# twosixlabs/csl-gan

Hardware: AMD Instinct MI355X
Metric: images/sec/GPU CelebA DCResNet dp_mode=gc bs=128 at 1/2/4/8 MI355X (higher is better)
Workload: dtype f32; 1 GPU; CelebA DCResNet D-step: dp_mode=gc -gcm adaptive-pl -nms 32, WGAN-GP on mean samples, 3x64x64; compute_dtype=fp32_auto, storage_dtype=fp32, launch=hip_graph, batch_per_gpu=128, global_batch=128, parallelism=dp1, materialize=ghost, grad_sample_dtype=fp32, fuse_passes=True

## Files before the change

csl_gan_amd/csrc/igemm_skinny.hip:

```cpp
#include "common.h"
#include "device_prims.h"
#include "igemm.h"
#include "conv_classes.h"

namespace cslgan {

constexpr int SK_MAXT = 9;
constexpr int SK_C = 64;
constexpr int SK_HALO = 12 * 12;

template <int NJ, bool ALL>
__global__ __launch_bounds__(256) void igemm_skinny_kernel(const KcParams p) {
    __shared__ float4 Hs[SK_HALO * 16];

    const int tid = threadIdx.x;
    const int b = xcd_remap(blockIdx.x, p.tiles_m);
    int ci = 0;
    if (!ALL) {
#pragma unroll 1
        while (ci + 1 < p.n_cls && b >= p.cls[ci + 1].tile0) ++ci;
    }
    const KcClass& kc = p.cls[ci];
    const int HW_ = kc.halo_w, hpix = kc.halo_h * kc.halo_w;
    const RowCoord rc0 = kc_decode_row((ALL ? b : b - kc.tile0) * 64, kc.OHc, kc.OWc, 1);
    const int y0 = rc0.oy + kc.ty_min, x0 = rc0.ox + kc.tx_min;
    const int img_base = rc0.img * p.AH * p.AW * SK_C;

    const __amdgpu_buffer_rsrc_t a_rsrc = make_rsrc(p.a, p.a_bytes);
    const int cl = tid & 15;
    if (p.a_bf16) {
        constexpr int HREG8 = (SK_HALO * 8 + 255) / 256;
        uint4 r8[HREG8];
#pragma unroll
        for (int j = 0; j < HREG8; ++j) {
            const int idx = tid + 256 * j;
            const int c8 = idx & 7, pix = idx >> 3;
            const int hy = pix / HW_, hx = pix - hy * HW_;
            const int iy = y0 + hy, ix = x0 + hx;
            const bool ok = pix < hpix && (unsigned)iy < (unsigned)p.VH && (unsigned)ix < (unsigned)p.VW;
            const auto v = buf_load4_raw(a_rsrc, (ok ? 2u * (unsigned)(img_base + (iy * p.AW + ix) * SK_C + c8 * 8) : BUF_OOB));
            r8[j] = make_uint4(v[0], v[1], v[2], v[3]);
        }
#pragma unroll
        for (int j = 0; j < HREG8; ++j) {
            const int idx = tid + 256 * j;
            if ((idx >> 3) < hpix) {
                const uint4 v = r8[j];
                Hs[2 * idx] = make_float4(bf_lo(v.x), bf_hi(v.x), bf_lo(v.y), bf_hi(v.y));
                Hs[2 * idx + 1] = make_float4(bf_lo(v.z), bf_hi(v.z), bf_lo(v.w), bf_hi(v.w));
            }
        }
    } else {
        constexpr int HREG = (SK_HALO * 16 + 255) / 256;
        float4 rh[HREG];
        unsigned okm = 0;
        const bool aff = p.in_scale != nullptr;
        float4 sc = make_float4(1.f, 1.f, 1.f, 1.f), sh = make_float4(0.f, 0.f, 0.f, 0.f);
        if (aff) {
            sc = *reinterpret_cast<const float4*>(p.in_scale + rc0.img * SK_C + cl * 4);
            sh = *reinterpret_cast<const float4*>(p.in_shift + rc0.img * SK_C + cl * 4);
        }
#pragma unroll
        for (int j = 0; j < HREG; ++j) {
            const int idx = tid + 256 * j;
            const int c4 = idx & 15, pix = idx >> 4;
            const int hy = pix / HW_, hx = pix - hy * HW_;
            const int iy = y0 + hy, ix = x0 + hx;
            const bool ok = pix < hpix && (unsigned)iy < (unsigned)p.VH && (unsigned)ix < (unsigned)p.VW;
            okm |= (ok ? 1u : 0u) << j;
            rh[j] = buf_load4(a_rsrc, ok ? 4u * (unsigned)(img_base + (iy * p.AW + ix) * SK_C + c4 * 4) : BUF_OOB);
        }
#pragma unroll
        for (int j = 0; j < HREG; ++j) {
            const int idx = tid + 256 * j;
            if (aff) {
                const float lo = p.in_relu ? 0.f : -__builtin_inff();
                const bool in = (okm >> j) & 1u;
                rh[j].x = in ? fmaxf(fmaf(sc.x, rh[j].x, sh.x), lo) : 0.f;
                rh[j].y = in ? fmaxf(fmaf(sc.y, rh[j].y, sh.y), lo) : 0.f;
                rh[j].z = in ? fmaxf(fmaf(sc.z, rh[j].z, sh.z), lo) : 0.f;
                rh[j].w = in ? fmaxf(fmaf(sc.w, rh[j].w, sh.w), lo) : 0.f;
            }
            if ((idx >> 4) < hpix) Hs[idx] = rh[j];
        }
    }
    __syncthreads();

    const int wid = tid >> 6, pg = (tid & 63) >> 4;
    float bv = 0.f;
    if (p.bias && cl < p.Nn) bv = p.bias[cl];
#pragma unroll 1
    for (int cc = ALL ? 0 : ci; cc < (ALL ? p.n_cls : ci + 1); ++cc) {
    const KcClass& kk = p.cls[cc];
    const int Tc = kk.T;
    const __amdgpu_buffer_rsrc_t w_rsrc = make_rsrc(p.w + kk.w_off, p.w_bytes - 4u * (unsigned)kk.w_off);
    float4 wr[SK_MAXT][NJ];
    int toff[SK_MAXT];
#pragma unroll
    for (int t = 0; t < SK_MAXT; ++t) {
        toff[t] = t < Tc ? (((int)kk.ty[t] - kk.ty_min) * HW_ + ((int)kk.tx[t] - kk.tx_min)) * 16 : 0;
#pragma unroll
        for (int j = 0; j < NJ; ++j)
            wr[t][j] = buf_load4(w_rsrc, (t < Tc && j < p.Nn) ? 4u * (unsigned)(j * kk.Kdim + t * SK_C + cl * 4) : BUF_OOB);
    }
#pragma unroll
    for (int it = 0; it < 4; ++it) {
        const int q = wid * 16 + it * 4 + pg;
        const int qy = q >> 3, qx = q & 7;
        const int base = (qy * HW_ + qx) * 16 + cl;
        float acc[NJ];
#pragma unroll
        for (int j = 0; j < NJ; ++j) acc[j] = 0.f;
#pragma unroll
        for (int t = 0; t < SK_MAXT; ++t) {
            if (t < Tc) {
                const float4 a = Hs[base + toff[t]];
#pragma unroll
                for (int j = 0; j < NJ; ++j) {
                    acc[j] = fmaf(a.x, wr[t][j].x, acc[j]);
                    acc[j] = fmaf(a.y, wr[t][j].y, acc[j]);
                    acc[j] = fmaf(a.z, wr[t][j].z, acc[j]);
                    acc[j] = fmaf(a.w, wr[t][j].w, acc[j]);
                }
            }
        }
#pragma unroll
        for (int j = 0; j < NJ; ++j) {
            acc[j] += __shfl_xor(acc[j], 1);
            acc[j] += __shfl_xor(acc[j], 2);
            acc[j] += __shfl_xor(acc[j], 4);
            acc[j] += __shfl_xor(acc[j], 8);
        }
        if (cl < p.Nn) {
            float val = acc[0];
#pragma unroll
            for (int j = 1; j < NJ; ++j) val = cl == j ? acc[j] : val;
            val += bv;
            const RowCoord rc = {rc0.img, rc0.oy + qy, rc0.ox + qx};
            const int off = kc_out_offset(p, kk, rc);
            if (p.res) val += p.res[kc_res_offset(p, kk, rc) + cl];
            val = apply_act(val, p.act);
            if (p.mask) val = lrelu_mask(val, p.mask[off + cl]);
            p.out[off + cl] = val;
        }
    }
    }
}

bool skinny_eligible(const KcParams& p) {
    if (p.Nn > 4 || p.Nn < 1 || p.sy != 1 || p.sx != 1 || p.AC != SK_C) return false;
    if (!aligned16(p.a) || !aligned16(p.w)) return false;
    for (int c = 0; c < p.n_cls; ++c) {
        const KcClass& k = p.cls[c];
        if (k.T < 1 || k.T > SK_MAXT || (k.OHc & 7) || (k.OWc & 7) || (k.M & 63) || (k.w_off & 3)) return false;
        int ymin, ymax, xmin, xmax;
        tap_range(k, ymin, ymax, xmin, xmax);
        if (ymax - ymin > 4 || xmax - xmin > 4) return false;
    }
    return true;
}

int launch_skinny(KcParams& p, hipStream_t st) {
    int tm = 0;
    for (int c = 0; c < p.n_cls; ++c) {
        KcClass& k = p.cls[c];
        int ymin, ymax, xmin, xmax;
        tap_range(k, ymin, ymax, xmin, xmax);
        k.ty_min = ymin; k.tx_min = xmin; k.halo_h = 8 + ymax - ymin; k.halo_w = 8 + xmax - xmin;
        k.patch = 1;
        k.tile0 = tm;
        tm += k.M / 64;
    }
    bool all = p.n_cls > 1;
    int uy0 = 127, uy1 = -128, ux0 = 127, ux1 = -128;
    for (int c = 0; c < p.n_cls; ++c) {
        const KcClass& k = p.cls[c];
        all = all && k.OHc == p.cls[0].OHc && k.OWc == p.cls[0].OWc && k.M == p.cls[0].M;
        uy0 = k.ty_min < uy0 ? k.ty_min : uy0; ux0 = k.tx_min < ux0 ? k.tx_min : ux0;
        uy1 = k.ty_min + k.halo_h > uy1 ? k.ty_min + k.halo_h : uy1; ux1 = k.tx_min + k.halo_w > ux1 ? k.tx_min + k.halo_w : ux1;
    }
    all = all && (uy1 - uy0) * (ux1 - ux0) <= SK_HALO;
    if (all) {
        for (int c = 0; c < p.n_cls; ++c) {
            KcClass& k = p.cls[c];
            k.ty_min = uy0; k.tx_min = ux0; k.halo_h = uy1 - uy0; k.halo_w = ux1 - ux0;
        }
        tm = p.cls[0].M / 64;
    }
    p.tiles_m = tm;
    p.tiles_n = 1;
    p.ksplit = 1;
    const dim3 grid((unsigned)tm), block(256);
    note_kernel("igemm_skinny_kernel<%d%s>", p.Nn < 4 ? p.Nn : 4, all ? ",all" : "");
#define CSL_SKINNY(NJ_)                                                                              \
    if (all) hipLaunchKernelGGL((igemm_skinny_kernel<NJ_, true>), grid, block, 0, st, p);            \
    else hipLaunchKernelGGL((igemm_skinny_kernel<NJ_, false>), grid, block, 0, st, p);
    switch (p.Nn) {
        case 1: CSL_SKINNY(1) break;
        case 2: CSL_SKINNY(2) break;
        case 3: CSL_SKINNY(3) break;
        default: CSL_SKINNY(4) break;
    }
#undef CSL_SKINNY
    return check_launch("igemm_skinny_kernel");
}


struct SkinnyWgradParams {
    const float* gy;
    const float* x;
    int N, H, W, P, Q, T, n_patches;
    unsigned x_bytes;
    float alpha;
    float* partial;
    signed char ty[SK_MAXT], tx[SK_MAXT];
    int ty_min, tx_min, halo_h, halo_w;
};

template <int NJ>
__global__ __launch_bounds__(256) void skinny_wgrad_kernel(const SkinnyWgradParams p) {
    __shared__ float4 Hs[SK_HALO * 16];
    __shared__ float Gs[64 * 4];
    const int tid = threadIdx.x;
    const int T = p.T, HW_ = p.halo_w, hpix = p.halo_h * p.halo_w;
    const int cl = tid & 15, wid = tid >> 6, pg = (tid & 63) >> 4;
    const __amdgpu_buffer_rsrc_t x_rsrc = make_rsrc(p.x, p.x_bytes);
    int toff[SK_MAXT];
#pragma unroll
    for (int t = 0; t < SK_MAXT; ++t) toff[t] = t < T ? (((int)p.ty[t] - p.ty_min) * HW_ + ((int)p.tx[t] - p.tx_min)) * 16 : 0;
    float4 acc[SK_MAXT][NJ];
#pragma unroll
    for (int t = 0; t < SK_MAXT; ++t)
#pragma unroll
        for (int j = 0; j < NJ; ++j) acc[t][j] = make_float4(0.f, 0.f, 0.f, 0.f);

    constexpr int HREG = (SK_HALO * 16 + 255) / 256;
    const int per_img = (p.P >> 3) * (p.Q >> 3);
    for (int pt = blockIdx.x; pt < p.n_patches; pt += gridDim.x) {
        const int img = pt / per_img, rem = pt - img * per_img;
        const int gyy = rem / (p.Q >> 3), gxx = rem - gyy * (p.Q >> 3);
        const int oy0 = gyy << 3, ox0 = gxx << 3;
        float4 rh[HREG];
#pragma unroll
        for (int j = 0; j < HREG; ++j) {
            const int idx = tid + 256 * j;
            const int c4 = idx & 15, pix = idx >> 4;
            const int hy = pix / HW_, hx = pix - hy * HW_;
            const int iy = oy0 + p.ty_min + hy, ix = ox0 + p.tx_min + hx;
            const bool ok = pix < hpix && (unsigned)iy < (unsigned)p.H && (unsigned)ix < (unsigned)p.W;
            rh[j] = buf_load4(x_rsrc, ok ? 4u * (unsigned)(((img * p.H + iy) * p.W + ix) * SK_C + c4 * 4) : BUF_OOB);
        }
        float gv = 0.f;
        if (tid < 64 * NJ) {
            const int q = tid / NJ, j = tid - q * NJ;
            gv = p.gy[((long long)(img * p.P + oy0 + (q >> 3)) * p.Q + ox0 + (q & 7)) * NJ + j];
        }
        __syncthreads();
#pragma unroll
        for (int j = 0; j < HREG; ++j) {
            const int idx = tid + 256 * j;
            if ((idx >> 4) < hpix) Hs[idx] = rh[j];
        }
        if (tid < 64 * NJ) Gs[(tid / NJ) * 4 + (tid % NJ)] = gv;
        __syncthreads();
#pragma unroll
        for (int it = 0; it < 4; ++it) {
            const int q = wid * 16 + it * 4 + pg;
            const int base = ((q >> 3) * HW_ + (q & 7)) * 16 + cl;
            float g[NJ];
#pragma unroll
            for (int j = 0; j < NJ; ++j) g[j] = Gs[q * 4 + j];
#pragma unroll
            for (int t = 0; t < SK_MAXT; ++t) {
                if (t < T) {
                    const float4 a = Hs[base + toff[t]];
#pragma unroll
                    for (int j = 0; j < NJ; ++j) {
                        acc[t][j].x = fmaf(g[j], a.x, acc[t][j].x);
                        acc[t][j].y = fmaf(g[j], a.y, acc[t][j].y);
                        acc[t][j].z = fmaf(g[j], a.z, acc[t][j].z);
                        acc[t][j].w = fmaf(g[j], a.w, acc[t][j].w);
                    }
                }
            }
        }
    }
    __syncthreads();
    float* red = reinterpret_cast<float*>(Hs);
#pragma unroll
    for (int t = 0; t < SK_MAXT; ++t) {
        if (t < T) {
#pragma unroll
            for (int j = 0; j < NJ; ++j) {
                float4 v = acc[t][j];
                v.x += __shfl_xor(v.x, 16); v.y += __shfl_xor(v.y, 16); v.z += __shfl_xor(v.z, 16); v.w += __shfl_xor(v.w, 16);
                v.x += __shfl_xor(v.x, 32); v.y += __shfl_xor(v.y, 32); v.z += __shfl_xor(v.z, 32); v.w += __shfl_xor(v.w, 32);
                if (pg == 0) *reinterpret_cast<float4*>(&red[((wid * NJ + j) * T + t) * 64 + cl * 4]) = v;
            }
        }
    }
    __syncthreads();
    const int n_out = NJ * T * 64;
    float* dst = p.partial + (long long)blockIdx.x * n_out;
    for (int i = tid; i < n_out; i += 256)
        dst[i] = p.alpha * (red[i] + red[n_out + i] + red[2 * n_out + i] + red[3 * n_out + i]);
}

}

using namespace cslgan;

extern "C" {

int cslgan_conv2d_wgrad_skinny_f32(const cslgan_conv_t* c, const float* gy, const float* x, float alpha, float* partial,
                                   int n_blocks, void* stream) {
    CSLGAN_REQUIRE(c && gy && x && partial, "conv2d_wgrad_skinny: null argument");
    CSLGAN_REQUIRE(c->K >= 1 && c->K <= 4 && c->C == SK_C, "conv2d_wgrad_skinny: needs 1..4 output and 64 input channels");
    CSLGAN_REQUIRE(c->stride == 1 && c->R * c->S <= SK_MAXT && c->R <= 5 && c->S <= 5, "conv2d_wgrad_skinny: needs stride 1 and at most 9 taps");
    CSLGAN_REQUIRE(c->N > 0 && c->P == c->H + 2 * c->pad - c->R + 1 && c->Q == c->W + 2 * c->pad - c->S + 1, "conv2d_wgrad_skinny: inconsistent output size");
    CSLGAN_REQUIRE((c->P & 7) == 0 && (c->Q & 7) == 0, "conv2d_wgrad_skinny: output grid must be a multiple of 8x8");
    CSLGAN_REQUIRE(n_blocks >= 1 && aligned16(x), "conv2d_wgrad_skinny: bad workspace / alignment");
    CSLGAN_REQUIRE(4ll * c->N * c->H * c->W * SK_C < (long long)BUF_OOB, "conv2d_wgrad_skinny: input larger than 4 GB");
    SkinnyWgradParams p{};
    p.gy = gy; p.x = x; p.N = c->N; p.H = c->H; p.W = c->W; p.P = c->P; p.Q = c->Q; p.T = c->R * c->S;
    p.n_patches = c->N * (c->P >> 3) * (c->Q >> 3);
    p.x_bytes = (unsigned)(4ll * c->N * c->H * c->W * SK_C);
    p.alpha = alpha; p.partial = partial;
    fill_forward_taps(p.ty, p.tx, c->R, c->S, c->pad);
    p.ty_min = -c->pad; p.tx_min = -c->pad; p.halo_h = 8 + c->R - 1; p.halo_w = 8 + c->S - 1;
    const dim3 grid((unsigned)n_blocks), block(256);
    note_kernel("skinny_wgrad_kernel<%d>", c->K);
    switch (c->K) {
        case 1: hipLaunchKernelGGL((skinny_wgrad_kernel<1>), grid, block, 0, (hipStream_t)stream, p); break;
        case 2: hipLaunchKernelGGL((skinny_wgrad_kernel<2>), grid, block, 0, (hipStream_t)stream, p); break;
        case 3: hipLaunchKernelGGL((skinny_wgrad_kernel<3>), grid, block, 0, (hipStream_t)stream, p); break;
        default: hipLaunchKernelGGL((skinny_wgrad_kernel<4>), grid, block, 0, (hipStream_t)stream, p); break;
    }
    return check_launch("skinny_wgrad_kernel");
}

}
```

Before: 19670 images/sec.

## Make fp32 skinny igemm persistent with prefetched halo and DPP reductions

After: 19850 images/sec, median of 6. About the same (+0.9%).

```diff
diff --git a/csl_gan_amd/csrc/igemm_skinny.hip b/csl_gan_amd/csrc/igemm_skinny.hip
--- a/csl_gan_amd/csrc/igemm_skinny.hip
+++ b/csl_gan_amd/csrc/igemm_skinny.hip
@@ -8,9 +8,214 @@
 constexpr int SK_MAXT = 9;
 constexpr int SK_C = 64;
 constexpr int SK_HALO = 12 * 12;
+constexpr int SK_HREG = SK_HALO * 16 / 256;
+constexpr int SK_GRID = 512;
+
+template <int CTRL>
+__device__ __forceinline__ float sk_dpp_add(float v) {
+    return v + __int_as_float(__builtin_amdgcn_update_dpp(0, __float_as_int(v), CTRL, 0xF, 0xF, false));
+}
+__device__ __forceinline__ float sk_row16_sum(float v) {
+    v = sk_dpp_add<0xB1>(v);
+    v = sk_dpp_add<0x4E>(v);
+    v = sk_dpp_add<0x141>(v);
+    v = sk_dpp_add<0x140>(v);
+    return v;
+}
+
+template <int N> struct SkTaps { static constexpr int value = N; };
 
 template <int NJ, bool ALL>
-__global__ __launch_bounds__(256) void igemm_skinny_kernel(const KcParams p) {
+__global__ __launch_bounds__(256, 2) void igemm_skinny_kernel(const KcParams p) {
+    __shared__ float4 Hs[SK_HALO * 16];
+    constexpr int NG = ALL ? 4 : 1;
+
+    const int tid = threadIdx.x;
+    const int cl = tid & 15, pg = (tid & 63) >> 4;
+    const int wid = __builtin_amdgcn_readfirstlane(tid >> 6);
+    const __amdgpu_buffer_rsrc_t a_rsrc = make_rsrc(p.a, p.a_bytes);
+    const bool aff = p.in_scale != nullptr;
+    const float lo = p.in_relu ? 0.f : -__builtin_inff();
+
+    const int oj = cl & 3, oq = (cl >> 2) * 4 + pg;
+    float bv = 0.f;
+    if (p.bias && oj < p.Nn) bv = p.bias[oj];
+
+    const int my_cls = ALL ? ((wid + (int)blockIdx.x) & 3) : 0;
+    const bool active = !ALL || my_cls < p.n_cls;
+
+#pragma unroll 1
+    for (int ci = 0; ci < (ALL ? 1 : p.n_cls); ++ci) {
+    const KcClass& kc = p.cls[ci];
+    const KcClass& kk = p.cls[ALL ? (active ? my_cls : 0) : ci];
+    const int n_patch = kc.M >> 6;
+    const int HW_ = kc.halo_w, hpix = kc.halo_h * kc.halo_w;
+    const unsigned rcp = (65536u + (unsigned)HW_ - 1u) / (unsigned)HW_;
+
+    f32x4 wr[SK_MAXT][NJ];
+    int toff[SK_MAXT];
+    const int Tc = active ? kk.T : 0;
+    {
+        const __amdgpu_buffer_rsrc_t w_rsrc = make_rsrc(p.w + kk.w_off, p.w_bytes - 4u * (unsigned)kk.w_off);
+#pragma unroll
+        for (int t = 0; t < SK_MAXT; ++t) {
+            toff[t] = t < Tc ? (((int)kk.ty[t] - kk.ty_min) * HW_ + ((int)kk.tx[t] - kk.tx_min)) * 16 : 0;
+#pragma unroll
+            for (int j = 0; j < NJ; ++j) {
+                const float4 v = buf_load4(w_rsrc, (t < Tc && j < p.Nn) ? 4u * (unsigned)(j * kk.Kdim + t * SK_C + cl * 4) : BUF_OOB);
+                wr[t][j] = f32x4{v.x, v.y, v.z, v.w};
+            }
+        }
+#pragma unroll
+        for (int t = 0; t < SK_MAXT; ++t)
+#pragma unroll
+            for (int j = 0; j < NJ; ++j) asm volatile("" : "+v"(wr[t][j]));
+    }
+    unsigned soff[SK_HREG];
+#pragma unroll
+    for (int j = 0; j < SK_HREG; ++j) {
+        const int idx = tid + 256 * j;
+        const int c4 = idx & 15, pix = idx >> 4;
+        const int hy = (int)(((unsigned)pix * rcp) >> 16), hx = pix - hy * HW_;
+        soff[j] = pix < hpix ? 4u * (unsigned)((hy * p.AW + hx) * SK_C + c4 * 4) : 0u;
+    }
+
+    float4 rh[SK_HREG];
+    unsigned okm = 0;
+    bool s_inner = false;
+    float4 sc = make_float4(1.f, 1.f, 1.f, 1.f), sh = make_float4(0.f, 0.f, 0.f, 0.f);
+    RowCoord s_rc = {0, 0, 0};
+    auto fetch = [&](int patch) {
+        const RowCoord rc = kc_decode_row(xcd_remap(patch, n_patch) * 64, kc.OHc, kc.OWc, 1);
+        s_rc = rc;
+        const int y0 = rc.oy + kc.ty_min, x0 = rc.ox + kc.tx_min;
+        const int img_base = rc.img * p.AH * p.AW * SK_C;
+        if (aff) {
+            sc = *reinterpret_cast<const float4*>(p.in_scale + rc.img * SK_C + cl * 4);
+            sh = *reinterpret_cast<const float4*>(p.in_shift + rc.img * SK_C + cl * 4);
+        }
+        s_inner = y0 >= 0 && x0 >= 0 && y0 + kc.halo_h <= p.VH && x0 + HW_ <= p.VW;
+        if (s_inner) {
+            const unsigned base = 4u * (unsigned)(img_base + (y0 * p.AW + x0) * SK_C);
+#pragma unroll
+            for (int j = 0; j < SK_HREG; ++j) rh[j] = buf_load4(a_rsrc, base + soff[j]);
+        } else {
+            okm = 0;
+#pragma unroll
+            for (int j = 0; j < SK_HREG; ++j) {
+                const int idx = tid + 256 * j;
+                int pix = idx >> 4;
+                asm volatile("" : "+v"(pix));
+                const int c4 = idx & 15;
+                const int hy = (int)(((unsigned)pix * rcp) >> 16), hx = pix - hy * HW_;
+                const int iy = y0 + hy, ix = x0 + hx;
+                const bool ok = pix < hpix && (unsigned)iy < (unsigned)p.VH && (unsigned)ix < (unsigned)p.VW;
+                okm |= (ok ? 1u : 0u) << j;
+                rh[j] = buf_load4(a_rsrc, ok ? 4u * (unsigned)(img_base + (iy * p.AW + ix) * SK_C + c4 * 4) : BUF_OOB);
+            }
+        }
+    };
+    auto commit = [&]() {
+#pragma unroll
+        for (int j = 0; j < SK_HREG; ++j) {
+            float4 v = rh[j];
+            if (aff) {
+                v.x = fmaxf(fmaf(sc.x, v.x, sh.x), lo);
+                v.y = fmaxf(fmaf(sc.y, v.y, sh.y), lo);
+                v.z = fmaxf(fmaf(sc.z, v.z, sh.z), lo);
+                v.w = fmaxf(fmaf(sc.w, v.w, sh.w), lo);
+                if (!s_inner && !((okm >> j) & 1u)) v = make_float4(0.f, 0.f, 0.f, 0.f);
+            }
+            Hs[tid + 256 * j] = v;
+        }
+    };
+
+    if ((int)blockIdx.x < n_patch) fetch(blockIdx.x);
+#pragma unroll 1
+    for (int pt = blockIdx.x; pt < n_patch; pt += gridDim.x) {
+        const RowCoord rc0 = s_rc;
+        __syncthreads();
+        commit();
+        __syncthreads();
+        unsigned mpos = 0;
+        if (p.mask && active && oj < p.Nn) {
+#pragma unroll
+            for (int g = 0; g < NG; ++g) {
+                const int q = (ALL ? g : wid) * 16 + oq;
+                const RowCoord rc = {rc0.img, rc0.oy + (q >> 3), rc0.ox + (q & 7)};
+                mpos |= (p.mask[kc_out_offset(p, kk, rc) + oj] > 0.f ? 1u : 0u) << g;
+            }
+        }
+        if (pt + (int)gridDim.x < n_patch) fetch(pt + gridDim.x);
+
+        auto run = [&](auto taps) {
+            constexpr int TT = decltype(taps)::value;
+#pragma unroll 1
+            for (int g = 0; g < NG; ++g) {
+                float val = 0.f;
+#pragma unroll 1
+                for (int it = 0; it < 4; ++it) {
+                    const int q = (ALL ? g : wid) * 16 + it * 4 + pg;
+                    const int base = ((q >> 3) * HW_ + (q & 7)) * 16 + cl;
+                    f32x2 acc[NJ];
+#pragma unroll
+                    for (int j = 0; j < NJ; ++j) acc[j] = f32x2{0.f, 0.f};
+                    if constexpr (TT > 0 && NJ == 3) {
+                        float4 a4[TT];
+#pragma unroll
+                        for (int t = 0; t < TT; ++t) a4[t] = Hs[base + toff[t]];
+                        __builtin_amdgcn_sched_barrier(0);
+#pragma unroll
+                        for (int t = 0; t < TT; ++t) {
+                            const f32x2 a01 = {a4[t].x, a4[t].y}, a23 = {a4[t].z, a4[t].w};
+#pragma unroll
+                            for (int j = 0; j < NJ; ++j) {
+                                acc[j] = __builtin_elementwise_fma(a01, wr[t][j].xy, acc[j]);
+                                acc[j] = __builtin_elementwise_fma(a23, wr[t][j].zw, acc[j]);
+                            }
+                        }
+                    } else {
+#pragma unroll
+                        for (int t = 0; t < SK_MAXT; ++t) {
+                            if (TT ? t < TT : t < Tc) {
+                                const float4 a4 = Hs[base + toff[t]];
+                                const f32x2 a01 = {a4.x, a4.y}, a23 = {a4.z, a4.w};
+#pragma unroll
+                                for (int j = 0; j < NJ; ++j) {
+                                    acc[j] = __builtin_elementwise_fma(a01, wr[t][j].xy, acc[j]);
+                                    acc[j] = __builtin_elementwise_fma(a23, wr[t][j].zw, acc[j]);
+                                }
+                            }
+                        }
+                    }
+#pragma unroll
+                    for (int j = 0; j < NJ; ++j) {
+                        const float s = sk_row16_sum(acc[j].x + acc[j].y);
+                        val = cl == it * 4 + j ? s : val;
+                    }
+                }
+                if (oj < p.Nn) {
+                    const int q = (ALL ? g : wid) * 16 + oq;
+                    const RowCoord rc = {rc0.img, rc0.oy + (q >> 3), rc0.ox + (q & 7)};
+                    const int off = kc_out_offset(p, kk, rc);
+                    val += bv;
+                    if (p.res) val += p.res[kc_res_offset(p, kk, rc) + oj];
+                    val = apply_act(val, p.act);
+                    if (p.mask) val *= (mpos >> g) & 1u ? 1.f : 0.2f;
+                    p.out[off + oj] = val;
+                }
+            }
+        };
+        if (Tc == 9) run(SkTaps<9>());
+        else if (Tc == 6) run(SkTaps<6>());
+        else if (Tc == 4) run(SkTaps<4>());
+        else if (Tc > 0) run(SkTaps<0>());
+    }
+    }
+}
+
+template <int NJ, bool ALL>
+__global__ __launch_bounds__(256) void igemm_skinny_bf16in_kernel(const KcParams p) {
     __shared__ float4 Hs[SK_HALO * 16];
 
     const int tid = threadIdx.x;
@@ -28,7 +233,7 @@
 
     const __amdgpu_buffer_rsrc_t a_rsrc = make_rsrc(p.a, p.a_bytes);
     const int cl = tid & 15;
-    if (p.a_bf16) {
+    {
         constexpr int HREG8 = (SK_HALO * 8 + 255) / 256;
         uint4 r8[HREG8];
 #pragma unroll
@@ -49,39 +254,6 @@
                 Hs[2 * idx] = make_float4(bf_lo(v.x), bf_hi(v.x), bf_lo(v.y), bf_hi(v.y));
                 Hs[2 * idx + 1] = make_float4(bf_lo(v.z), bf_hi(v.z), bf_lo(v.w), bf_hi(v.w));
             }
-        }
-    } else {
-        constexpr int HREG = (SK_HALO * 16 + 255) / 256;
-        float4 rh[HREG];
-        unsigned okm = 0;
-        const bool aff = p.in_scale != nullptr;
-        float4 sc = make_float4(1.f, 1.f, 1.f, 1.f), sh = make_float4(0.f, 0.f, 0.f, 0.f);
-        if (aff) {
-            sc = *reinterpret_cast<const float4*>(p.in_scale + rc0.img * SK_C + cl * 4);
-            sh = *reinterpret_cast<const float4*>(p.in_shift + rc0.img * SK_C + cl * 4);
-        }
-#pragma unroll
-        for (int j = 0; j < HREG; ++j) {
-            const int idx = tid + 256 * j;
-            const int c4 = idx & 15, pix = idx >> 4;
-            const int hy = pix / HW_, hx = pix - hy * HW_;
-            const int iy = y0 + hy, ix = x0 + hx;
-            const bool ok = pix < hpix && (unsigned)iy < (unsigned)p.VH && (unsigned)ix < (unsigned)p.VW;
-            okm |= (ok ? 1u : 0u) << j;
-            rh[j] = buf_load4(a_rsrc, ok ? 4u * (unsigned)(img_base + (iy * p.AW + ix) * SK_C + c4 * 4) : BUF_OOB);
-        }
-#pragma unroll
-        for (int j = 0; j < HREG; ++j) {
-            const int idx = tid + 256 * j;
-            if (aff) {
-                const float lo = p.in_relu ? 0.f : -__builtin_inff();
-                const bool in = (okm >> j) & 1u;
-                rh[j].x = in ? fmaxf(fmaf(sc.x, rh[j].x, sh.x), lo) : 0.f;
-                rh[j].y = in ? fmaxf(fmaf(sc.y, rh[j].y, sh.y), lo) : 0.f;
-                rh[j].z = in ? fmaxf(fmaf(sc.z, rh[j].z, sh.z), lo) : 0.f;
-                rh[j].w = in ? fmaxf(fmaf(sc.w, rh[j].w, sh.w), lo) : 0.f;
-            }
-            if ((idx >> 4) < hpix) Hs[idx] = rh[j];
         }
     }
     __syncthreads();
@@ -190,10 +362,13 @@
     p.tiles_m = tm;
     p.tiles_n = 1;
     p.ksplit = 1;
-    const dim3 grid((unsigned)tm), block(256);
+    const dim3 grid((unsigned)(tm < SK_GRID ? tm : SK_GRID)), block(256);
     note_kernel("igemm_skinny_kernel<%d%s>", p.Nn < 4 ? p.Nn : 4, all ? ",all" : "");
-#define CSL_SKINNY(NJ_)                                                                              \
-    if (all) hipLaunchKernelGGL((igemm_skinny_kernel<NJ_, true>), grid, block, 0, st, p);            \
+    const dim3 grid1((unsigned)tm);
+#define CSL_SKINNY(NJ_)                                                                                                       \
+    if (p.a_bf16 && all) hipLaunchKernelGGL((igemm_skinny_bf16in_kernel<NJ_, true>), grid1, block, 0, st, p);                 \
+    else if (p.a_bf16) hipLaunchKernelGGL((igemm_skinny_bf16in_kernel<NJ_, false>), grid1, block, 0, st, p);                  \
+    else if (all) hipLaunchKernelGGL((igemm_skinny_kernel<NJ_, true>), grid, block, 0, st, p);                                \
     else hipLaunchKernelGGL((igemm_skinny_kernel<NJ_, false>), grid, block, 0, st, p);
     switch (p.Nn) {
         case 1: CSL_SKINNY(1) break;
```
